# hardcamls/video-coding

Measured on AMD Instinct MI355X. Metric: Mpixel/s decoded (1080p 4:2:0 batch), higher is better.
Workload: dtype int32

## Files before the change

### video-coding_amd/csrc/hvc_capi_reader.hip

```cpp
#include "hvc_batch.h"

static bool same_geometry(const hvc_jpeg_info &a, const hvc_jpeg_info &b) {
    if (a.n_comp != b.n_comp || a.coef_count != b.coef_count || a.width != b.width || a.height != b.height ||
        std::memcmp(a.layout, b.layout, sizeof a.layout))
        return false;
    for (int i = 0; i < a.n_comp; i++) {
        const hvc_jpeg_component &x = a.comp[i], &y = b.comp[i];
        if (x.identifier != y.identifier || x.hscale != y.hscale || x.vscale != y.vscale || x.decoded_width != y.decoded_width ||
            x.decoded_height != y.decoded_height || x.actual_width != y.actual_width || x.actual_height != y.actual_height)
            return false;
    }
    return true;
}

static bool gd_geometry(const hvc_jpeg_info &info0, hvc::HdParams &P) {
    std::memset(&P, 0, sizeof P);
    if (info0.n_comp < 1 || info0.n_comp > 3) return false;
    P.n_comp = info0.n_comp;
    const hvc_jpeg_component &c0 = info0.comp[0];
    if (c0.hscale < 1 || c0.vscale < 1) return false;
    P.mbs_wide = c0.decoded_width / (8 * c0.hscale);
    P.mbs_high = c0.decoded_height / (8 * c0.vscale);
    int base = 0;
    for (int i = 0; i < info0.n_comp; i++) {
        P.comp[i].h = info0.comp[i].hscale;
        P.comp[i].v = info0.comp[i].vscale;
        P.comp[i].bw = info0.layout[i].blocks_w;
        P.comp[i].mcu_base = base;
        P.comp[i].coef_off = info0.layout[i].coef_offset;
        if (P.comp[i].h < 1 || P.comp[i].v < 1) return false;
        if (P.mbs_wide * P.comp[i].h > info0.layout[i].blocks_w || P.mbs_high * P.comp[i].v > info0.layout[i].blocks_h)
            return false;
        if (base + P.comp[i].h * P.comp[i].v > HVC_HD_MAX_MCU_BLOCKS) return false;
        for (int k = 0; k < P.comp[i].h * P.comp[i].v; k++) P.b2comp[base + k] = (unsigned char)i;
        base += P.comp[i].h * P.comp[i].v;
    }
    P.blocks_per_mcu = base;
    const unsigned long long bpf = (unsigned long long)P.mbs_wide * P.mbs_high * base;
    if (bpf == 0 || bpf >= (1ull << 31) || info0.coef_count >= (1ull << 32)) return false;
    P.blocks_per_frame = (unsigned)bpf;
    return true;
}

static void gd_carve_state(hvc::HdParams &P, void *mem, size_t n) {
    unsigned long long *sp = (unsigned long long *)mem;
    P.start_used = sp;
    P.exit_a = sp + n;
    P.exit_b = sp + 2 * n;
    P.exit_c = sp + 3 * n;
    unsigned *up = (unsigned *)(sp + 4 * n);
    P.nblk = up;
    P.list0 = up + n;
    P.list1 = up + 2 * n;
    P.list_n = up + 3 * n;
}

static int gd_upload_tables(hvc_ctx *c, const hvc::HdTables &t, hvc::HdParams &P, hipStream_t st) {
    int r;
    if ((r = grow(c, c->gd_tables, sizeof(hvc::HdTables) + sizeof(hvc::HdSpec) + sizeof(hvc::HdSpecOvf)))) return r;
    hvc::HdSpec spec;
    hvc::HdSpecOvf spec_ovf;
    unsigned char slot[4];
    static const bool classic = std::getenv("HVC_HD_CLASSIC") != nullptr;
    const bool have_spec = hvc::make_spec(t, P.n_comp, spec, slot, P.slot_rep, &spec_ovf) && !classic;
    if (!c->gd_tables_host) c->gd_tables_host.reset(new (std::nothrow) hvc::HdTables);
    if (!c->gd_tables_host) return HVC_E_OUT_OF_MEMORY;
    if (!(c->gd_tables_valid && c->gd_tables_ncomp == P.n_comp && !std::memcmp(c->gd_tables_host.get(), &t, sizeof t))) {
        c->gd_tables_valid = false;
        HIPCHK(c, hipMemcpyAsync(c->gd_tables.p, &t, sizeof t, hipMemcpyHostToDevice, st));
        if (have_spec) {
            HIPCHK(c, hipMemcpyAsync(c->gd_tables.as<char>() + sizeof t, &spec, sizeof spec, hipMemcpyHostToDevice, st));
            HIPCHK(c, hipMemcpyAsync(c->gd_tables.as<char>() + sizeof t + sizeof spec, &spec_ovf, sizeof spec_ovf, hipMemcpyHostToDevice, st));
        }
        HIPCHK(c, hipStreamSynchronize(st));
        std::memcpy(c->gd_tables_host.get(), &t, sizeof t);
        c->gd_tables_ncomp = P.n_comp;
        c->gd_tables_valid = true;
    }
    P.tables = c->gd_tables.as<const hvc::HdTables>();
    P.spec = have_spec ? (const hvc::HdSpec *)(c->gd_tables.as<char>() + sizeof t) : nullptr;
    P.spec_ovf = have_spec ? (const hvc::HdSpecOvf *)(c->gd_tables.as<char>() + sizeof t + sizeof(hvc::HdSpec)) : nullptr;
    P.ftabs = nullptr;
    P.tabset_of = nullptr;
    P.slotmask = P.selmask = 0;
    for (int b = 0; b < P.blocks_per_mcu; b++) {
        P.slotmask |= (unsigned)slot[P.b2comp[b]] << b;
        P.selmask |= (unsigned)slot[P.b2comp[b]] << (2 * b);
    }
    return HVC_OK;
}

static bool gd_lists_per_frame(size_t total_sub, int n_frames) {
    return n_frames >= 1 && n_frames <= 65535 && total_sub / (size_t)n_frames >= 1024;
}

static unsigned gd_component_selmask(const hvc::HdParams &P) {
    unsigned m = 0;
    for (int b = 0; b < P.blocks_per_mcu; b++) m |= (unsigned)P.b2comp[b] << (2 * b);
    return m;
}

static hipError_t gd_enqueue(const hvc::HdParams &P, int rounds, hipStream_t st) {
    hipError_t e = hvc::launch_hd_frame_of(P, st);
    for (int r = 0; r < rounds && e == hipSuccess; r++) e = hvc::launch_hd_round(P, r, st);
    if (e == hipSuccess) e = hvc::launch_hd_finish(P, rounds, st);
    return e;
}
static bool gd_unsettled(unsigned changed_word, int rounds) { return rounds > 1 && changed_word == (unsigned)(rounds - 1); }

static bool call_timing() {
    static const bool on = std::getenv("HVC_CALL_TIMING") != nullptr;
    return on;
}
struct StageClock {
    std::chrono::steady_clock::time_point t0 = std::chrono::steady_clock::now(), last = t0;
    char line[512];
    int n = 0;
    void mark(const char *what) {
        if (!call_timing()) return;
        const auto now = std::chrono::steady_clock::now();
        n += std::snprintf(line + n, sizeof line - (size_t)n, " %s %.1f", what, std::chrono::duration<double, std::micro>(now - last).count());
        if (n > (int)sizeof line - 64) n = (int)sizeof line - 64;
        last = now;
    }
    void done() {
        if (!call_timing()) return;
        std::fprintf(stderr, "hvc call timing (us):%s | total %.1f\n", line, std::chrono::duration<double, std::micro>(last - t0).count());
    }
};

int gpu_entropy_decode(hvc_ctx *c, const uint8_t *const *jpegs, const size_t *sizes, int n_frames, const hvc_jpeg_info &info0,
                       int16_t *d_coefs, size_t coef_fs, int *used_gpu, AfterReader *after) {
    *used_gpu = 0;
    if (after) after->speculated = false;
    StageClock clk;
    std::vector<hvc::HdTables> sets;
    hvc::HdParams P;
// ... 133 lines not shown
        }
        for (size_t k = 0; k < sets.size(); k++) hvc::make_frame_tabs(sets[k], P.n_comp, ftabs[k]);
        const size_t tb = sets.size() * sizeof(hvc::HdFrameTabs);
        if ((r = grow(c, c->gd_ftabs, tb + nU * sizeof(unsigned)))) return r;
        HIPCHK(c, hipMemcpyAsync(c->gd_ftabs.p, ftabs.data(), tb, hipMemcpyHostToDevice, st));
        HIPCHK(c, hipMemcpyAsync(c->gd_ftabs.as<char>() + tb, tabset_of.data(), nU * sizeof(unsigned), hipMemcpyHostToDevice, st));
        P.tables = nullptr;
        P.spec = nullptr;
        P.ftabs = c->gd_ftabs.as<const hvc::HdFrameTabs>();
        P.tabset_of = (const unsigned *)(c->gd_ftabs.as<char>() + tb);
        P.selmask = gd_component_selmask(P);
        if (gd_lists_per_frame(P.total_sub, n_frames)) {
            if ((r = grow(c, c->gd_fcnt, (size_t)HVC_HD_LIST_N * nU * sizeof(unsigned)))) return r;
            P.list_fn = c->gd_fcnt.as<unsigned>();
            for (size_t f = 0; f < (size_t)n_frames; f++) P.max_frame_sub = std::max(P.max_frame_sub, sub_off[(f + 1) * ipf] - sub_off[f * ipf]);
        }
    }
    P.ecs = c->gd_ecs.as<const uint8_t>();
    P.ecs_off = d_ecs_off;
    P.sub_off = d_sub_off;
    P.frame_of = d_frame_of;
    P.coefs = d_coefs;
    P.coef_fs = coef_fs;
    gd_carve_state(P, c->gd_state.p, subs);
    P.frame_blocks = d_frame_blocks;
    P.changed = d_flags;
    P.status = d_flags + 1;
    if (after && after->dc_plane) {
        P.dc_plane = after->dc_plane;
        P.dc_fs = after->dc_fs;
    }
    clk.mark("uploads-enqueued");
    const int first_rounds = 4;
    HIPCHK(c, gd_enqueue(P, first_rounds, st));
    clk.mark("reader-enqueued");
    bool consumer_enqueued = false;
    if (after && after->enqueue) {
        if ((r = after->enqueue())) return r;
        consumer_enqueued = true;
    }
    clk.mark("consumer-enqueued");
    unsigned flags[2] = {0, 0};
    HIPCHK(c, hipMemcpyAsync(flags, P.changed, sizeof flags, hipMemcpyDeviceToHost, st));
    HIPCHK(c, hipStreamSynchronize(st));
    clk.mark("synchronised");
    clk.done();
#ifdef HVC_HD_STATS
    {
        unsigned ln[HVC_HD_LIST_N];
        HIPCHK(c, hipMemcpy(ln, P.list_n, sizeof ln, hipMemcpyDeviceToHost));
        std::fprintf(stderr, "hd stats: %u subsequences; lists", P.total_sub);
        for (int q = 2; q < HVC_HD_LIST_N - 2; q++) std::fprintf(stderr, " %u", ln[q]);
        std::fprintf(stderr, "; k_hd_round walks %u, inner rounds %u; changed %u status %u\n", ln[HVC_HD_LIST_N - 2], ln[HVC_HD_LIST_N - 1], flags[0], flags[1]);
        unsigned long long hs[4];
        hvc::hd_stats_read(hs);
        std::fprintf(stderr, "hd stats: round 0 walked %llu symbols (%.1f a subsequence); 64 x the longest walk of every wavefront: %llu (lanes busy %.1f %%)\n",
                     hs[0], (double)hs[0] / P.total_sub, hs[1], 100.0 * (double)hs[0] / (double)(hs[1] ? hs[1] : 1));
        const unsigned long long own = hs[2] & 0xffffffffull, over = hs[2] >> 32;
        std::fprintf(stderr, "hd stats: write pass %llu symbols inside the lanes' own subsequences + %llu beyond them (%.1f %%); 64 x trips of every wavefront: %llu (lanes busy %.1f %%)\n",
                     own, over, 100.0 * (double)over / (double)(own ? own : 1), hs[3], 100.0 * (double)(own + over) / (double)(hs[3] ? hs[3] : 1));
    }
#endif
    if (gd_unsettled(flags[0], first_rounds)) {
        consumer_enqueued = false;
        const int max_rounds = 48;
        int round = 0;
        HIPCHK(c, hvc::launch_hd_frame_of(P, st));
        for (;; round++) {
            HIPCHK(c, hvc::launch_hd_round(P, round, st));
            if (round >= 4) {
                unsigned changed = 0;
                HIPCHK(c, hipMemcpyAsync(&changed, P.changed, sizeof changed, hipMemcpyDeviceToHost, st));
                HIPCHK(c, hipStreamSynchronize(st));
                if (!gd_unsettled(changed, round + 1)) break;
                if (round >= max_rounds) return HVC_OK;
            }
        }
        HIPCHK(c, hvc::launch_hd_finish(P, round + 1, st));
        HIPCHK(c, hipMemcpyAsync(flags + 1, P.status, sizeof(unsigned), hipMemcpyDeviceToHost, st));
        HIPCHK(c, hipStreamSynchronize(st));
    }
    const unsigned status = flags[1];
    static const bool hd_debug = std::getenv("HVC_HD_DEBUG") != nullptr;
    if (hd_debug) std::fprintf(stderr, "hd debug: frames %d subs %u changed %u status %u\n", P.n_frames, P.total_sub, flags[0], status);
    if (status) return HVC_OK;
    *used_gpu = 1;
    if (after) after->speculated = consumer_enqueued;
    return HVC_OK;
}

int hvc_jpeg_entropy_decode_gpu(hvc_ctx *c, const uint8_t *const *jpegs, const size_t *sizes, int n_frames, int16_t *coefs,
                                size_t coef_fs, int where, hvc_jpeg_info *info, int *used_gpu) try {
    if (!c || !jpegs || !sizes || !coefs || !info || n_frames < 1) return HVC_E_INVALID_ARG;
    if (where != HVC_MEM_HOST && where != HVC_MEM_DEVICE) return HVC_E_INVALID_ARG;
    hvc::RestartScope honour(c->honour_restart);
    int r = hvc_jpeg_read_header(jpegs[0], sizes[0], info);
    if (r) return r;
    if ((n_frames > 1 && coef_fs < info->coef_count) || (coef_fs & 7)) return HVC_E_INVALID_ARG;
    DeviceGuard g(c->device);
    if (!g.ok) return fail_hip(c, hipErrorInvalidDevice);
    int16_t *d = coefs;
    const size_t total = ((size_t)(n_frames - 1) * coef_fs + info->coef_count) * sizeof(int16_t);
    if (where == HVC_MEM_HOST) {
        if ((r = grow(c, c->gd_coefs, total))) return r;
        d = c->gd_coefs.as<int16_t>();
    } else if ((uintptr_t)coefs & 15) {
        return HVC_E_ALIGNMENT;
    }
    int gpu = 0;
    r = gpu_entropy_decode(c, jpegs, sizes, n_frames, *info, d, coef_fs, &gpu);
    if (r) return r;
    if (used_gpu) *used_gpu = gpu;
    if (gpu) {
        if (where == HVC_MEM_HOST) {
            for (int f = 0; f < n_frames; f++)
                HIPCHK(c, hipMemcpyAsync(coefs + (size_t)f * coef_fs, d + (size_t)f * coef_fs, info->coef_count * sizeof(int16_t),
                                         hipMemcpyDeviceToHost, c->stream));
            HIPCHK(c, hipStreamSynchronize(c->stream));
        }
        return HVC_OK;
    }
    std::vector<int16_t> tmp;
    for (int f = 0; f < n_frames; f++) {
        hvc_jpeg_info fi;
        if ((r = hvc_jpeg_read_header(jpegs[f], sizes[f], &fi))) return r;
        if (fi.coef_count != info->coef_count || std::memcmp(fi.layout, info->layout, sizeof fi.layout)) return HVC_E_INVALID_ARG;
        if (where == HVC_MEM_HOST) {
            if ((r = hvc_jpeg_entropy_decode(jpegs[f], sizes[f], &fi, coefs + (size_t)f * coef_fs))) return r;
        } else {
            tmp.resize(info->coef_count);
            if ((r = hvc_jpeg_entropy_decode(jpegs[f], sizes[f], &fi, tmp.data()))) return r;
            HIPCHK(c, hipMemcpyAsync(coefs + (size_t)f * coef_fs, tmp.data(), info->coef_count * sizeof(int16_t),
                                     hipMemcpyHostToDevice, c->stream));
            HIPCHK(c, hipStreamSynchronize(c->stream));
        }
    }
    return HVC_OK;
} HVC_ABI_CATCH

int decode_batch_gpu(hvc_ctx *c, const uint8_t *const *jpegs, const size_t *sizes, int n_frames, int threads, int frames_per_chunk,
                     uint8_t *pixels, size_t pixel_fs, int where, hvc_batch_stats *stats, OutputForm form) {
    if (!c || !jpegs || !sizes || !pixels || n_frames < 0) return HVC_E_INVALID_ARG;
    if (!form.known()) return HVC_E_INVALID_ARG;
    if (where != HVC_MEM_HOST && where != HVC_MEM_DEVICE) return HVC_E_INVALID_ARG;
    if (stats) std::memset(stats, 0, sizeof *stats);
    if (n_frames == 0) return HVC_OK;
    hvc::RestartScope honour(c->honour_restart);
    auto host_pipeline = [&]() {
        return decode_batch_impl(c, jpegs, sizes, n_frames, threads, frames_per_chunk, pixels, pixel_fs, where, stats, form);
    };
    hvc_jpeg_info info0;
    int r = hvc_jpeg_read_header(jpegs[0], sizes[0], &info0);
    if (r) return r;
    form.of(info0);
    if ((r = form.batch_check(pixel_fs))) return r;
    const size_t out_bytes = form.out_bytes;
    hvc::HdParams G;
    hvc::HdTables tables0;
    const unsigned SB = HVC_HD_SUBSEQ_BITS / 8;
    unsigned rst = 0, ipf = 1;
    {
        const bool geo = gd_geometry(info0, G);
        if (geo && hvc::tl_honour_restart) {
            rst = hvc::restart_interval_of(jpegs[0], sizes[0]);
            const unsigned long long mcus = (unsigned long long)G.mbs_wide * (unsigned long long)G.mbs_high;
            if (rst && mcus > rst) {
                const unsigned long long q = (mcus + rst - 1) / rst;
// ... 366 lines not shown
```

### video-coding_amd/csrc/hvc_hdec.h

```cpp
#ifndef HVC_HDEC_H
#define HVC_HDEC_H

#include <hip/hip_runtime.h>
#include <stddef.h>
#include <stdint.h>

#include <vector>

struct hvc_jpeg_info;

namespace hvc {

#define HVC_HD_SUBTABLES 8
#define HVC_HD_OVF 0x3ffu

struct HdTable {
    uint16_t fast[1024];
    uint16_t sub[HVC_HD_SUBTABLES * 64];
};
struct HdOvfRaw {
    uint16_t mincode[6], count[6], valptr[6];
    uint8_t vals[256];
    uint8_t lens[256];
    uint16_t used, pad;
};
struct HdTables {
    HdTable dc[3], ac[3];
    HdOvfRaw ovf_dc[3], ovf_ac[3];
};
struct HdOvf {
    uint16_t mincode[6], count[6], valptr[6], pad[2];
    uint16_t spec[256];
    uint16_t val[256];
};

struct HdSpec {
    uint16_t t[2][2][1024 + HVC_HD_SUBTABLES * 64];
};
struct HdSpecOvf {
    HdOvf o[2][2];
};
bool make_spec(const HdTables &t, int n_comp, HdSpec &out, unsigned char slot_of_comp[4], unsigned char slot_rep[2],
               HdSpecOvf *ovf = nullptr);
bool tables_use_overflow(const HdTables &t, int n_comp);

#define HVC_HD_SPEC_T (1024 + HVC_HD_SUBTABLES * 64)
struct HdFrameTabs {
    uint16_t spec[3][2][HVC_HD_SPEC_T];
    uint16_t val[3][2][HVC_HD_SPEC_T];
    unsigned flags, pad[3];
    HdOvf ovf[3][2];
};
void make_frame_tabs(const HdTables &t, int n_comp, HdFrameTabs &out);

#ifndef HVC_HD_SUBSEQ_BITS
#define HVC_HD_SUBSEQ_BITS 1024
#endif
#define HVC_HD_MAX_MCU_BLOCKS 16
#define HVC_HD_ECS_SLACK 1024
#define HVC_HD_LIST_N 32
#define HVC_HD_STATE_BYTES(n) ((size_t)(n) * (4 * sizeof(unsigned long long) + 3 * sizeof(unsigned)) + HVC_HD_LIST_N * sizeof(unsigned) + 64)

struct HdComp {
    int h, v, bw;
    int mcu_base;
    size_t coef_off;
};

struct HdParams {
    const uint8_t *ecs;
    const unsigned *ecs_off;
    const unsigned *sub_off;
    const unsigned *frame_of;
    const HdTables *tables;
    const HdSpec *spec;
    const HdSpecOvf *spec_ovf;
    const HdFrameTabs *ftabs;
    const unsigned *tabset_of;
    unsigned selmask;
    unsigned slotmask;
    unsigned char slot_rep[2];
    int n_frames;
    unsigned total_sub;
    int n_comp, blocks_per_mcu, mbs_wide, mbs_high;
    unsigned blocks_per_frame;
    unsigned rst_mcus, rst_ipf;
    HdComp comp[4];
    unsigned char b2comp[HVC_HD_MAX_MCU_BLOCKS];
    int16_t *coefs;
    size_t coef_fs;
    unsigned long long *start_used, *exit_a, *exit_b;
    unsigned long long *exit_c;
    unsigned *list0, *list1, *list_n;
    unsigned *list_fn;
    unsigned max_frame_sub;
    int16_t *dcd;
    int16_t *dc_plane;
    size_t dc_fs;
    unsigned *nblk;
    unsigned *frame_blocks;
    unsigned *changed;
    unsigned *status;
};

hipError_t launch_hd_round(const HdParams &P, int round, hipStream_t s);
#ifdef HVC_HD_STATS
void hd_stats_read(unsigned long long out[4]);
#endif
hipError_t launch_hd_frame_of(const HdParams &P, hipStream_t s);
hipError_t launch_hd_finish(const HdParams &P, int rounds_done, hipStream_t s);
bool hd_write2_fits(const HdParams &P);
inline unsigned hd_files(const HdParams &P) { return P.rst_ipf > 1 ? ((unsigned)P.n_frames + P.rst_ipf - 1) / P.rst_ipf : (unsigned)P.n_frames; }

int prepare_gpu_decode(const uint8_t *jpeg, size_t n, const ::hvc_jpeg_info *info, HdTables &t, std::vector<uint8_t> &ecs,
                       bool &gpu_ok);
struct RstUnits {
    unsigned interval, ipf;
    unsigned *off, *len;
};
inline size_t hd_unit_subs(size_t len) { return len ? (len + HVC_HD_SUBSEQ_BITS / 8 - 1) / (HVC_HD_SUBSEQ_BITS / 8) : 1; }
inline size_t hd_unit_slot(size_t len) { return hd_unit_subs(len) * (HVC_HD_SUBSEQ_BITS / 8) + 16; }
int prepare_gpu_decode_to(const uint8_t *jpeg, size_t n, const ::hvc_jpeg_info *info, HdTables &t, uint8_t *dst, size_t cap,
                          size_t *ecs_size, bool &gpu_ok, RstUnits *units = nullptr);
unsigned restart_interval_of(const uint8_t *jpeg, size_t n);


struct WideDc {
    uint32_t block;
    long long dc;
};
extern thread_local bool tl_honour_restart;
struct RestartScope {
    bool prev;
    explicit RestartScope(bool on) : prev(tl_honour_restart) { tl_honour_restart = on; }
    ~RestartScope() { tl_honour_restart = prev; }
};
int entropy_decode_wide(const uint8_t *data, size_t n, const ::hvc_jpeg_info *info, int16_t *coefs, std::vector<WideDc> &wide);
void entropy_decode_wide2(const uint8_t *const data[2], const size_t n[2], const ::hvc_jpeg_info *const info[2], int16_t *const coefs[2],
                          std::vector<WideDc> *const wide[2], int st[2]);

}
#endif
```

### video-coding_amd/csrc/hvc_hdec.hip

```cpp
#include "hvc_hdec_dev.h"

#include <cstdlib>
#include <cstring>
#include <type_traits>

namespace hvc {

using namespace hd_dev;

namespace {

__device__ __forceinline__ bool hd_unsettled(const HdParams &P, int rounds_done) {
    return rounds_done > 1 && *P.changed == (unsigned)(rounds_done - 1);
}

struct FrameRef {
    unsigned file, mcu0, need;
};
__device__ __forceinline__ FrameRef frame_ref(const HdParams &P, unsigned f) {
    FrameRef r{f, 0u, P.blocks_per_frame};
    if (P.rst_ipf > 1u) {
        r.file = f / P.rst_ipf;
        r.mcu0 = (f - r.file * P.rst_ipf) * P.rst_mcus;
        const unsigned left = (unsigned)P.mbs_wide * (unsigned)P.mbs_high - r.mcu0;
        r.need = (left < P.rst_mcus ? left : P.rst_mcus) * (unsigned)P.blocks_per_mcu;
    }
    return r;
}

__device__ __forceinline__ bool one_file(const HdParams &P, unsigned f0, unsigned f1) {
    return f0 == f1 || (P.rst_ipf > 1u && f0 / P.rst_ipf == f1 / P.rst_ipf);
}

__device__ __forceinline__ unsigned be32(const unsigned *g, unsigned i) { return __builtin_bswap32(g[i]); }

__device__ __forceinline__ unsigned lookup(const HdTable &t, unsigned long long w) {
    unsigned e = t.fast[(unsigned)(w >> 54)];
    if (e & 0x8000u) e = t.sub[(e & 0x7fffu) * 64u + ((unsigned)(w >> 48) & 63u)];
    return e;
}

__device__ __forceinline__ int extend(int cat, unsigned code) {
    return (code & (1u << (cat - 1))) ? (int)code : (int)code - (int)((1u << cat) - 1);
}

struct HdGeo {
    int h[4], v[4], bw[4], mcu_base[4];
    unsigned coef_off[4];
    unsigned char b2comp[HVC_HD_MAX_MCU_BLOCKS], b2sx[HVC_HD_MAX_MCU_BLOCKS], b2sy[HVC_HD_MAX_MCU_BLOCKS];
};
__device__ __forceinline__ void load_geo(const HdParams &P, HdGeo &G) {
    if (threadIdx.x < 4) {
        const int i = threadIdx.x;
        G.h[i] = P.comp[i].h;
        G.v[i] = P.comp[i].v;
        G.bw[i] = P.comp[i].bw;
        G.mcu_base[i] = P.comp[i].mcu_base;
        G.coef_off[i] = (unsigned)P.comp[i].coef_off;
    }
    if (threadIdx.x < HVC_HD_MAX_MCU_BLOCKS) {
        const int bb = threadIdx.x, comp = P.b2comp[bb];
        const int r = bb - P.comp[comp].mcu_base, hh = P.comp[comp].h > 0 ? P.comp[comp].h : 1;
        G.b2comp[bb] = (unsigned char)comp;
        G.b2sy[bb] = (unsigned char)(r >= 0 ? r / hh : 0);
        G.b2sx[bb] = (unsigned char)(r >= 0 ? r % hh : 0);
    }
}

template <bool WRITE>
__device__ __forceinline__ void walk(const HdParams &P, const HdGeo &G, const HdTables &T, const unsigned *slot, unsigned base, unsigned limit,
                                     unsigned &p, int &k, int &b, unsigned &nb, unsigned first_block, int16_t *rec,
                                     unsigned &err, int16_t *lb = nullptr, unsigned mcu0 = 0u, unsigned need = 0u) {
    const int B = P.blocks_per_mcu;
    unsigned bi = first_block;
    int16_t *blk = nullptr;
    int lo = k;
    unsigned mx = 0, my = 0;
    if (WRITE) {
        const unsigned mcu = first_block / (unsigned)B + mcu0;
        my = mcu / (unsigned)P.mbs_wide;
        mx = mcu - my * (unsigned)P.mbs_wide;
    }
    auto block_ptr = [&](int bb) -> int16_t * {
        const int comp = G.b2comp[bb];
        return rec + G.coef_off[comp] +
               ((size_t)(my * (unsigned)G.v[comp] + G.b2sy[bb]) * (unsigned)G.bw[comp] + (size_t)(mx * (unsigned)G.h[comp] + G.b2sx[bb])) * 64;
    };
    bool live = WRITE && bi < need;
    if (live) blk = block_ptr(b);
    unsigned off = p - base;
    unsigned wi = (off >> 5) + 2;
    unsigned long long buf = (((unsigned long long)be32(slot, off >> 5) << 32) | be32(slot, (off >> 5) + 1)) << (off & 31u);
    int avail = 64 - (int)(off & 31u);
    unsigned n0 = be32(slot, wi), n1 = be32(slot, min(wi + 1, (unsigned)(S / 32 + 3)));
    int comp = G.b2comp[b];
    const HdTable *dct = &T.dc[comp], *act = &T.ac[comp];
// ... 30 lines not shown
        buf <<= used;
        avail -= used;
        p += (unsigned)used;
        bool end_block = false;
        if (is_dc) {
            if (live) {
                lb[0] = (int16_t)mag;
                if (mag < -32768 || mag > 32767) err |= 2u;
            }
            k = 1;
        } else if (mag == 0 && run == 0) {
            end_block = true;
        } else {
            k += run;
            if (k >= 64) {
                if (live) err |= 1u;
                end_block = true;
            } else {
                if (live && mag) lb[k] = (int16_t)mag;
                k++;
                end_block = k == 64;
            }
        }
        if (end_block) {
            if (live) {
                if (lo == 0) {
                    const uint4 z = make_uint4(0, 0, 0, 0);
#pragma unroll
                    for (int q = 0; q < 8; q++) {
                        reinterpret_cast<uint4 *>(blk)[q] = reinterpret_cast<const uint4 *>(lb)[q];
                        reinterpret_cast<uint4 *>(lb)[q] = z;
                    }
                } else {
                    for (int q = lo; q < 64; q++) {
                        blk[q] = lb[q];
                        lb[q] = 0;
                    }
                }
            }
            lo = 0;
            k = 0;
            b = b + 1 == B ? 0 : b + 1;
            nb++;
            bi++;
            comp = G.b2comp[b];
            dct = &T.dc[comp];
            act = &T.ac[comp];
            if (WRITE && b == 0) {
                mx++;
                if (mx == (unsigned)P.mbs_wide) {
                    mx = 0;
                    my++;
                }
            }
            live = WRITE && bi < need;
            if (live) blk = block_ptr(b);
        }
    }
    if (live)
        for (int q = lo; q < k; q++) blk[q] = lb[q];
}

}


#ifdef HVC_HD_STATS
__device__ unsigned long long g_hd_stats[4];
void hd_stats_read(unsigned long long out[4]) {
    unsigned long long z[4] = {0, 0, 0, 0};
    (void)hipMemcpyFromSymbol(out, HIP_SYMBOL(g_hd_stats), sizeof z);
    (void)hipMemcpyToSymbol(HIP_SYMBOL(g_hd_stats), z, sizeof z);
}
#endif

constexpr int INNER = 24;
template <int MODE>
__global__ __launch_bounds__(256) void k_hd_round(HdParams P, int round) {
    constexpr bool PF = MODE == 2;
    __shared__ __attribute__((aligned(16))) unsigned char Traw[MODE == 0 ? sizeof(HdTables) : sizeof(HdSpec)];
    __shared__ unsigned rows[MODE != 0 ? 256 * SROW + 2 : 1];
    HdTables &T = *reinterpret_cast<HdTables *>(Traw);
    __shared__ HdGeo G;
    __shared__ unsigned long long exits[256];
    load_geo(P, G);
    const int tid = threadIdx.x;
    const unsigned i = blockIdx.x * 256u + (unsigned)tid;
    const bool valid = i < P.total_sub;
    const unsigned f = valid ? P.frame_of[i] : 0u, j = valid ? i - P.sub_off[f] : 0u;
    const unsigned *slot = reinterpret_cast<const unsigned *>(P.ecs + P.ecs_off[f] + (size_t)j * (S / 8));
    const unsigned long long *prev = (round & 1) ? P.exit_a : P.exit_b;
    unsigned long long *cur = (round & 1) ? P.exit_b : P.exit_a;
    const unsigned base = j * (unsigned)S;
    unsigned long long st = pack_state(base, 0, 0), used = 0, ex = 0;
    bool have = false;
    unsigned nb = 0;
    if (valid && round > 0) {
        used = P.start_used[i];
        ex = prev[i];
        nb = P.nblk[i];
        have = true;
        if (j > 0) st = prev[i - 1];
    }
    bool pf_lds = false;
    if (__syncthreads_or(valid && (!have || st != used))) {
        const unsigned *src = MODE == 1 ? reinterpret_cast<const unsigned *>(P.spec) : reinterpret_cast<const unsigned *>(P.tables);
        if (PF) {
            const unsigned i0 = blockIdx.x * 256u, i1 = min(i0 + 256u, P.total_sub) - 1u;
            const unsigned f0 = P.frame_of[i0];
            if (one_file(P, f0, P.frame_of[i1])) {
                const HdFrameTabs &ft = P.ftabs[P.tabset_of[f0]];
                pf_lds = (ft.flags & 1u) != 0u;
                src = reinterpret_cast<const unsigned *>(&ft.spec[0][0][0]);
            }
        }
        if (!PF || pf_lds) {
            unsigned *dst = reinterpret_cast<unsigned *>(Traw);
            for (unsigned q = threadIdx.x; q < sizeof(Traw) / 4; q += 256) dst[q] = src[q];
        }
        __syncthreads();
    }
    bool changed = false;
    for (int inner = 0; inner < INNER; inner++) {
        if (valid && (!have || st != used)) {
            unsigned p = (unsigned)st, err = 0;
            int k = (int)((st >> 32) & 0xffu), b = (int)((st >> 40) & 0xffu);
            nb = 0;
            if (MODE != 0) {
                unsigned *row = rows + tid * SROW;
                stage_row(row, reinterpret_cast<const uint8_t *>(slot));
                auto rd = [row](unsigned q) { return row[q]; };
                const uint16_t *lt = reinterpret_cast<const uint16_t *>(Traw);
                if (MODE == 1) spec_walk<true, true>(rd, row, lt, &P.spec_ovf->o[0][0], P.slotmask, P.blocks_per_mcu, base, p, k, b, nb);
                else if (pf_lds) spec_walk<true, false>(rd, row, lt, &P.ftabs[P.tabset_of[f]].ovf[0][0], selmask_c2_as_c1(P.selmask), P.blocks_per_mcu, base, p, k, b, nb);
                else spec_walk<true, false>(rd, row, &P.ftabs[P.tabset_of[f]].spec[0][0][0], &P.ftabs[P.tabset_of[f]].ovf[0][0], P.selmask, P.blocks_per_mcu, base, p, k, b, nb);
            } else {
                walk<false>(P, G, T, slot, base, base + (unsigned)S, p, k, b, nb, 0, nullptr, err);
            }
            ex = pack_state(p, k, b);
            used = st;
            have = true;
            changed = true;
#ifdef HVC_HD_STATS
            if (round > 0) {
                atomicAdd(&P.list_n[HVC_HD_LIST_N - 2], 1u);
                atomicMax(&P.list_n[HVC_HD_LIST_N - 1], (unsigned)inner + 1u);
            }
#endif
        }
        exits[tid] = ex;
        __syncthreads();
        bool again = false;
        if (valid && j > 0 && tid > 0) {
            st = exits[tid - 1];
            again = st != used;
        }
        if (!__syncthreads_or(again)) break;
    }
    if (valid) {
        cur[i] = ex;
        P.start_used[i] = used;
        P.nblk[i] = nb;
        if (changed && round > 0) *P.changed = (unsigned)round;
    }
}

constexpr int SYNC_ROUNDS = 12, SYNC_ROUNDS_PF = 22;
// ... 97 lines not shown
    const unsigned f = g * ipf, f_end = min(f + ipf, (unsigned)P.n_frames), s0 = P.sub_off[f];
    const unsigned count = round < 2 ? P.sub_off[f_end] - s0 : P.list_fn[(unsigned)round * n_groups + g];
    if (blockIdx.x * (unsigned)SYNC_WG >= count) return;
    const HdFrameTabs &ft = P.ftabs[P.tabset_of[f]];
    const bool pf_lds = (ft.flags & 1u) != 0u;
    if (pf_lds) {
        const unsigned *src = reinterpret_cast<const unsigned *>(&ft.spec[0][0][0]);
        unsigned *dst = reinterpret_cast<unsigned *>(sp);
        for (unsigned i = threadIdx.x; i < sizeof(sp) / 4; i += SYNC_WG) dst[i] = src[i];
        __syncthreads();
    }
    const int wave = threadIdx.x >> 6, lane = threadIdx.x & 63;
    unsigned *row = rows[wave] + lane * SROW;
    const unsigned *list = ((round & 1) ? P.list1 : P.list0) + s0;
    unsigned *next = ((round & 1) ? P.list0 : P.list1) + s0;
    unsigned *next_n = P.list_fn + (unsigned)(round + 1) * n_groups + g;
    const unsigned long long *pe = (round & 1) ? P.exit_b : P.exit_c;
    unsigned long long *ce = (round & 1) ? P.exit_c : P.exit_b;
    int trip = 0;
    for (unsigned tb = blockIdx.x * (unsigned)SYNC_WG; tb < count; tb += gridDim.x * (unsigned)SYNC_WG, trip ^= 1) {
        const unsigned t = tb + (unsigned)threadIdx.x;
        const bool valid = t < count;
        const unsigned i = !valid ? s0 : round < 2 ? s0 + t : list[t];
        const bool push = sync_one<true>(P, round, valid, i, row, sp, pe, ce, pf_lds);
        const unsigned long long m = __ballot(push);
        if (round == 0) continue;
        if (lane == 0) wcount[trip][wave] = (unsigned)__popcll(m);
        __syncthreads();
        if (threadIdx.x == 0) {
            unsigned total = 0;
            for (int q = 0; q < SYNC_WG / 64; q++) total += wcount[trip][q];
            wbase[trip] = total ? atomicAdd(next_n, total) : 0u;
        }
        __syncthreads();
        unsigned at = wbase[trip];
        for (int q = 0; q < wave; q++) at += wcount[trip][q];
        if (push) next[at + (unsigned)__popcll(m & ((1ull << lane) - 1ull))] = i + 1;
    }
}

template <bool PF>
__global__ __launch_bounds__(SYNC_WG) void k_hd_sync_tail(HdParams P, int first_round, int last_round) {
    __shared__ uint16_t sp[PF ? 2 : 2 * 2 * SPEC_T];
    __shared__ unsigned rows[SYNC_WG / 64][64 * SROW + 2];
    __shared__ unsigned cnt_s[2];
    if (!PF) {
        const unsigned *src = reinterpret_cast<const unsigned *>(P.spec);
        unsigned *dst = reinterpret_cast<unsigned *>(sp);
        for (unsigned i = threadIdx.x; i < sizeof(HdSpec) / 4; i += SYNC_WG) dst[i] = src[i];
    }
    if (threadIdx.x == 0) {
        cnt_s[first_round & 1] = P.list_n[first_round];
        cnt_s[(first_round + 1) & 1] = 0;
    }
    __syncthreads();
    const int wave = threadIdx.x >> 6, lane = threadIdx.x & 63;
    unsigned *row = rows[wave] + lane * SROW;
    for (int round = first_round; round <= last_round; round++) {
        const unsigned count = cnt_s[round & 1];
        if (count == 0) break;
        const unsigned *list = (round & 1) ? P.list1 : P.list0;
        unsigned *next = (round & 1) ? P.list0 : P.list1;
        const unsigned long long *pe = (round & 1) ? P.exit_b : P.exit_c;
        unsigned long long *ce = (round & 1) ? P.exit_c : P.exit_b;
        for (unsigned t0 = (unsigned)wave * 64u; t0 < count; t0 += (unsigned)SYNC_WG) {
            const unsigned t = t0 + (unsigned)lane;
            const bool valid = t < count;
            const unsigned i = valid ? list[t] : 0u;
            const bool push = sync_one<PF>(P, round, valid, i, row, sp, pe, ce);
            const unsigned long long m = __ballot(push);
            if (m) {
                unsigned at = 0;
                if (lane == 0) at = atomicAdd(&cnt_s[(round + 1) & 1], (unsigned)__popcll(m));
                at = __shfl(at, 0);
                if (push) next[at + (unsigned)__popcll(m & ((1ull << lane) - 1ull))] = i + 1;
            }
        }
        __syncthreads();
        if (threadIdx.x == 0) cnt_s[round & 1] = 0;
        __syncthreads();
    }
}

__global__ __launch_bounds__(1024) void k_hd_scan(HdParams P) {
    __shared__ unsigned wsum[16];
    __shared__ unsigned carry_s;
    const int frame = blockIdx.x, lane = threadIdx.x, wave = lane >> 6, wl = lane & 63;
    unsigned *d = P.nblk + P.sub_off[frame];
    const unsigned n = P.sub_off[frame + 1] - P.sub_off[frame];
    if (lane == 0) carry_s = 0;
    __syncthreads();
    for (unsigned base = 0; base < n; base += 1024) {
        const unsigned idx = base + (unsigned)lane;
        const unsigned v = idx < n ? d[idx] : 0u;
        unsigned incl = v;
#pragma unroll
        for (int o = 1; o < 64; o <<= 1) {
            const unsigned t = __shfl_up(incl, o);
            if (wl >= o) incl += t;
        }
        if (wl == 63) wsum[wave] = incl;
        __syncthreads();
        unsigned wbase = 0;
        for (int q = 0; q < wave; q++) wbase += wsum[q];
        const unsigned excl = carry_s + wbase + incl - v;
        if (idx < n) d[idx] = excl;
        __syncthreads();
        if (lane == 1023) carry_s = excl + v;
        __syncthreads();
    }
    if (lane == 0) {
        P.frame_blocks[frame] = carry_s;
        if (carry_s < frame_ref(P, (unsigned)frame).need) atomicOr(P.status, 4u);
    }
}

__global__ __launch_bounds__(256) void k_hd_write(HdParams P, int final_round) {
    __shared__ HdTables T;
    __shared__ HdGeo G;
    __shared__ uint4 lbuf[256 * 8];
    load_geo(P, G);
    {
        const unsigned *src = reinterpret_cast<const unsigned *>(P.tables);
        unsigned *dst = reinterpret_cast<unsigned *>(&T);
        for (unsigned i = threadIdx.x; i < sizeof(HdTables) / 4; i += 256) dst[i] = src[i];
#pragma unroll
        for (int q = 0; q < 8; q++) lbuf[threadIdx.x * 8 + q] = make_uint4(0, 0, 0, 0);
    }
    const unsigned i = blockIdx.x * 256u + threadIdx.x;
    const bool valid = i < P.total_sub;
    const unsigned f = valid ? P.frame_of[i] : 0u, j = valid ? i - P.sub_off[f] : 0u;
    const unsigned *slot = reinterpret_cast<const unsigned *>(P.ecs + P.ecs_off[f] + (size_t)j * (S / 8));
    __syncthreads();
    if (hd_unsettled(P, final_round)) return;
    if (!valid) return;
    const unsigned first_block = P.nblk[i];
    const FrameRef R = frame_ref(P, f);
    if (first_block >= R.need) return;
    const unsigned long long st = P.start_used[i];
    unsigned p = (unsigned)st;
    int k = (int)((st >> 32) & 0xffu), b = (int)((st >> 40) & 0xffu);
    unsigned nb = 0, err = 0;
    if ((unsigned)b != first_block % (unsigned)P.blocks_per_mcu) {
        atomicOr(P.status, 8u);
        return;
    }
    const unsigned base = j * (unsigned)S;
    walk<true>(P, G, T, slot, base, base + (unsigned)S, p, k, b, nb, first_block, P.coefs + (size_t)R.file * P.coef_fs, err,
               reinterpret_cast<int16_t *>(lbuf + threadIdx.x * 8), R.mcu0, R.need);
    const unsigned long long *fin = (final_round & 1) ? P.exit_a : P.exit_b;
    if (pack_state(p, k, b) != fin[i]) err |= 8u;
    if (err) atomicOr(P.status, err);
}

constexpr int WR_EXTRA = 3;
#ifndef HVC_WR_BATCH
#define HVC_WR_BATCH 12
#endif
constexpr int WR_BATCH = HVC_WR_BATCH;

template <bool PF, bool GBITS, int WG>
__global__ __launch_bounds__(WG) void k_hd_write2(HdParams P, int final_round) {
    __shared__ uint16_t tv[2 * 2 * SPEC_T];
    __shared__ HdGeo G;
    __shared__ unsigned rows[GBITS ? 1 : (WG + WR_EXTRA + 2) * SROW];
    __shared__ uint4 lbuf[WG * 8];
    __shared__ uint2 flist[WG / 64][64];
    load_geo(P, G);
    {
        for (int sl = 0; sl < (PF ? 0 : 2); sl++)
            for (int cls = 0; cls < 2; cls++) {
                const HdTable *src_t = cls ? &P.tables->ac[P.slot_rep[sl]] : &P.tables->dc[P.slot_rep[sl]];
                const uint16_t *src = reinterpret_cast<const uint16_t *>(src_t);
                for (unsigned i = threadIdx.x; i < sizeof(HdTable) / 2; i += WG) tv[(sl * 2 + cls) * SPEC_T + i] = (uint16_t)val_entry(src[i], cls == 0, i >= 1024u);
            }
#pragma unroll
        for (int q = 0; q < 8; q++) lbuf[threadIdx.x * 8 + q] = make_uint4(0, 0, 0, 0);
    }
    const int tid = threadIdx.x, wave = tid >> 6, lane = tid & 63;
    const unsigned i = blockIdx.x * (unsigned)WG + (unsigned)tid;
    const bool valid = i < P.total_sub;
    const unsigned f = valid ? P.frame_of[i] : 0u, j = valid ? i - P.sub_off[f] : 0u;
    if (hd_unsettled(P, final_round)) return;
    bool pf_lds = false;
    if (PF) {
        const unsigned i0 = blockIdx.x * (unsigned)WG, i1 = min(i0 + (unsigned)WG, P.total_sub) - 1u;
        const unsigned f0 = P.frame_of[i0];
        if (one_file(P, f0, P.frame_of[i1])) {
            const HdFrameTabs &ft = P.ftabs[P.tabset_of[f0]];
            if (ft.flags & 1u) {
                pf_lds = true;
                const unsigned *src = reinterpret_cast<const unsigned *>(&ft.val[0][0][0]);
                unsigned *dst = reinterpret_cast<unsigned *>(tv);
                for (unsigned q = threadIdx.x; q < sizeof(tv) / 4; q += WG) dst[q] = src[q];
            }
        }
    }
    if (!GBITS) {
        if (valid) stage_row(rows + tid * SROW, P.ecs + P.ecs_off[f] + (size_t)j * (S / 8));
        if (tid < WR_EXTRA) {
            const unsigned i2 = blockIdx.x * (unsigned)WG + (unsigned)WG + (unsigned)tid;
            if (i2 < P.total_sub) {
                const unsigned f2 = P.frame_of[i2];
                stage_row(rows + (WG + tid) * SROW, P.ecs + P.ecs_off[f2] + (size_t)(i2 - P.sub_off[f2]) * (S / 8));
            }
        }
    }
    __syncthreads();
    const unsigned *row = rows + (GBITS ? 0 : tid * SROW);
    const unsigned *gbits = reinterpret_cast<const unsigned *>(P.ecs + P.ecs_off[f] + (size_t)j * (S / 8));
    auto rd = [&](unsigned q) -> unsigned { return GBITS ? __builtin_bswap32(gbits[q]) : row[q + (q ? (q - 1u) >> 5 : 0u)]; };
    auto rd1 = [&](unsigned q) -> unsigned { return GBITS ? __builtin_bswap32(gbits[q]) : row[q + ((q - 1u) >> 5)]; };
    static_assert(S == 1024, "rd(): S / 32 dwords per row");
    int16_t *const nowhere = reinterpret_cast<int16_t *>(&flist[wave][lane]);
    int16_t *const lb = reinterpret_cast<int16_t *>(lbuf + tid * 8);
    const int B = P.blocks_per_mcu;
    const unsigned base = j * (unsigned)S, limit = base + (unsigned)S, hard = limit + (unsigned)(WR_EXTRA * S);
    unsigned bi = valid ? P.nblk[i] : 0xffffffffu;
    const FrameRef R = frame_ref(P, f);
    bool act = valid && bi < R.need;
    const unsigned long long st = act ? P.start_used[i] : 0ull;
    const unsigned p0 = act ? (unsigned)st : base;
    int k = (int)((st >> 32) & 0xffu), b = (int)((st >> 40) & 0xffu);
    unsigned err = 0;
    if (act && (unsigned)b != bi % (unsigned)B) {
        err |= 8u;
        act = false;
    }
    bool live = act && k == 0;
    const unsigned mcu = (act ? bi : 0u) / (unsigned)B + R.mcu0;
    unsigned my = mcu / (unsigned)P.mbs_wide, mx = mcu - my * (unsigned)P.mbs_wide;
    const unsigned frame_unit0 = (unsigned)(((size_t)R.file * P.coef_fs) >> 3);
    auto block_no = [&](int bb) -> unsigned {
        const int comp = G.b2comp[bb];
        return frame_unit0 + (G.coef_off[comp] >> 3) +
               ((my * (unsigned)G.v[comp] + G.b2sy[bb]) * (unsigned)G.bw[comp] + (mx * (unsigned)G.h[comp] + G.b2sx[bb])) * 8u;
    };
    unsigned mm = ~(p0 - base + 31u);
    const unsigned l0 = (p0 - base + 31u) >> 5;
    unsigned hi = l0 ? rd(l0 - 1u) : 0u, lo = rd(l0), nx = rd(l0 + 1u);
    auto pos = [&]() -> unsigned { return base + ~mm - 31u; };
    auto mm_of = [&](unsigned p) -> unsigned { return ~(p - base + 31u); };
    auto decode_and_store = [&](const uint16_t *const tvb, const HdOvf *const ovf, const unsigned selmask) {
    const uint16_t *bt = tvb + ((selmask >> (2 * b)) & 3u) * (2 * SPEC_T);
    const uint16_t *bt_ac = bt + SPEC_T;
    const unsigned long long fin_i = valid ? ((final_round & 1) ? P.exit_a : P.exit_b)[i] : 0ull;
    const unsigned mm_limit = mm_of(limit), mm_hard = mm_of(hard);
    unsigned watch = mm_limit;
    unsigned cur_block = live ? block_no(b) : 0u;
#ifdef HVC_HD_STATS
    unsigned st_sym = 0, st_trips = 0;
#endif
    while (__any(act)) {
        unsigned npend = 0;
        if (act) for (;;) {
            const unsigned w = __builtin_amdgcn_alignbit(hi, lo, mm);
            const uint16_t *t = k ? bt_ac : bt;
            const HdSymbol sy = val_symbol(w, t, ovf, selmask, b, k);
            const unsigned used = sy.used;
            const int kn = sy.kn;
            const bool wrong = sy.wrong, end_block = sy.end_block;
            *((live && !wrong) ? lb + kn - 1 : nowhere) = (int16_t)sy.mag;
            k = end_block ? 64 : kn;
            const unsigned mn = mm - used;
            const bool refill = ((mn ^ mm) >> 5) != 0u;
            mm = mn;
            if (!GBITS) {
                hi = refill ? lo : hi;
                lo = refill ? nx : lo;
                nx = rd1((31u - mn) >> 5);
            } else if (refill) {
                hi = lo;
                lo = nx;
                nx = rd1((31u - mn) >> 5);
            }
            if ((live && wrong) || mm <= watch) {
                if (live && wrong) atomicOr(P.status, 1u);
                if (mm <= watch) {
                    if (watch == mm_limit) {
                        if (pack_state(pos(), end_block ? 0 : k, end_block ? (b + 1 == B ? 0 : b + 1) : b) != fin_i) atomicOr(P.status, 8u);
                        watch = mm_hard;
                        if (!end_block && !live) k = 65;
                    } else {
                        atomicOr(P.status, 1u);
                        k = 65;
                    }
                }
            }
            npend += (unsigned)__popcll(__ballot(k == 64));
#ifdef HVC_HD_STATS
            st_sym += mm > mm_limit ? 1u : 0x10000u;
            st_trips += (unsigned)__popcll(__ballot(true)) ? 1u : 0u;
#endif
            if (k >= 64 || npend >= (unsigned)WR_BATCH) break;
        }
        if (k == 65) act = false;
        const bool pending = act && k == 64;
        if (__any(pending)) {
            const bool flush = pending && live;
            const unsigned long long m = __ballot(flush);
            asm volatile("" ::: "memory");
            const unsigned n = (unsigned)__popcll(m);
            if (flush) {
                flist[wave][__popcll(m & ((1ull << lane) - 1ull))] = make_uint2(cur_block, (unsigned)(wave * 64 + lane));
                P.dcd[(size_t)f * P.blocks_per_frame + bi] = lb[0];
            }
            for (unsigned g = 0; g < n; g += 8) {
                const unsigned en = g + ((unsigned)lane >> 3);
                if (en < n) {
                    const uint2 fe = flist[wave][en];
                    uint4 *src = lbuf + fe.y * 8u + ((unsigned)lane & 7u);
                    reinterpret_cast<uint4 *>(P.coefs)[(size_t)fe.x + ((unsigned)lane & 7u)] = *src;
                    *src = make_uint4(0, 0, 0, 0);
                }
            }
            asm volatile("" ::: "memory");
            if (pending) {
                k = 0;
                b = b + 1 == B ? 0 : b + 1;
                bi++;
                live = bi < R.need;
                bt = tvb + ((selmask >> (2 * b)) & 3u) * (2 * SPEC_T);
                bt_ac = bt + SPEC_T;
                if (b == 0) {
                    mx++;
                    if (mx == (unsigned)P.mbs_wide) {
                        mx = 0;
                        my++;
                    }
// ... 99 lines not shown
        if (val) val[q] = (uint16_t)val_entry(e, dc, q >= 1024);
    }
}

static void convert_ovf(const HdOvfRaw &src, bool dc, HdOvf &o) {
    std::memset(&o, 0, sizeof o);
    for (int i = 0; i < 6; i++) {
        o.mincode[i] = src.mincode[i];
        o.count[i] = src.used ? src.count[i] : (uint16_t)0;
        o.valptr[i] = src.valptr[i];
    }
    for (int k = 0; k < 256; k++) {
        const unsigned len = src.lens[k], v = src.vals[k];
        uint16_t sp = 1, vl = 1;
        if (len) {
            const HdTable *none = nullptr;
            (void)none;
            const unsigned e = (len << 8) | v;
            if (dc) sp = (uint16_t)(v > 16 ? len : (len + v) | (1u << 6));
            else {
                const unsigned size = v & 15u, run = v >> 4;
                sp = (!size && !run) ? (uint16_t)(len | (64u << 6)) : (uint16_t)((len + size) | ((run + 1u) << 6));
            }
            vl = (uint16_t)val_entry(e, dc, true);
        }
        o.spec[k] = sp;
        o.val[k] = vl;
    }
}

bool tables_use_overflow(const HdTables &t, int n_comp) {
    for (int c = 0; c < n_comp && c < 3; c++)
        if (t.ovf_dc[c].used || t.ovf_ac[c].used) return true;
    return false;
}

bool make_spec(const HdTables &t, int n_comp, HdSpec &out, unsigned char slot_of_comp[4], unsigned char slot_rep[2], HdSpecOvf *ovf) {
    if (n_comp < 1 || n_comp > 3) return false;
    int rep[2] = {0, -1};
    for (int c = 0; c < 4; c++) slot_of_comp[c] = 0;
    for (int c = 1; c < n_comp; c++) {
        auto same = [&](int a) { return !std::memcmp(&t.dc[c], &t.dc[a], sizeof(HdTable)) && !std::memcmp(&t.ac[c], &t.ac[a], sizeof(HdTable)); };
        if (same(rep[0])) continue;
        if (rep[1] < 0) rep[1] = c;
        if (!same(rep[1])) return false;
        slot_of_comp[c] = 1;
    }
    slot_rep[0] = 0;
    slot_rep[1] = (unsigned char)(rep[1] < 0 ? 0 : rep[1]);
    std::memset(&out, 0, sizeof out);
    if (ovf) std::memset(ovf, 0, sizeof *ovf);
    for (int sl = 0; sl < 2; sl++) {
        if (rep[sl] < 0) continue;
        convert_table(t.dc[rep[sl]], true, out.t[sl][0], nullptr);
        convert_table(t.ac[rep[sl]], false, out.t[sl][1], nullptr);
        if (ovf) {
            convert_ovf(t.ovf_dc[rep[sl]], true, ovf->o[sl][0]);
            convert_ovf(t.ovf_ac[rep[sl]], false, ovf->o[sl][1]);
        }
    }
    return true;
}

void make_frame_tabs(const HdTables &t, int n_comp, HdFrameTabs &out) {
    out.flags = (n_comp < 3 || (!std::memcmp(&t.dc[2], &t.dc[1], sizeof(HdTable)) && !std::memcmp(&t.ac[2], &t.ac[1], sizeof(HdTable)))) ? 1u : 0u;
    out.pad[0] = out.pad[1] = out.pad[2] = 0;
    for (int c = 0; c < 3; c++) {
        const int s = c < n_comp ? c : 0;
        convert_table(t.dc[s], true, out.spec[c][0], out.val[c][0]);
        convert_table(t.ac[s], false, out.spec[c][1], out.val[c][1]);
        convert_ovf(t.ovf_dc[s], true, out.ovf[c][0]);
        convert_ovf(t.ovf_ac[s], false, out.ovf[c][1]);
    }
}

__global__ __launch_bounds__(256) void k_hd_frame_of(HdParams P) {
    const unsigned f = blockIdx.x, end = P.sub_off[f + 1];
    unsigned *frame_of = const_cast<unsigned *>(P.frame_of);
    for (unsigned q = P.sub_off[f] + threadIdx.x; q < end; q += 256u) frame_of[q] = f;
    if (f == 0) {
        if (threadIdx.x < HVC_HD_LIST_N) P.list_n[threadIdx.x] = 0u;
        if (threadIdx.x == 0) {
            *P.changed = 0u;
            *P.status = 0u;
        }
    }
    if (P.list_fn && threadIdx.x < HVC_HD_LIST_N) P.list_fn[threadIdx.x * (unsigned)P.n_frames + f] = 0u;
}

hipError_t launch_hd_frame_of(const HdParams &P, hipStream_t s) {
    if (P.total_sub == 0 || P.n_frames <= 0) return hipSuccess;
    hipLaunchKernelGGL(k_hd_frame_of, dim3((unsigned)P.n_frames), dim3(256), 0, s, P);
    return hipGetLastError();
}

template <bool PF>
static hipError_t launch_hd_round_t(const HdParams &P, int round, hipStream_t s) {
    if (round == 0 && (PF || P.spec)) {
        const unsigned all = (P.total_sub + (unsigned)SYNC_WG - 1u) / (unsigned)SYNC_WG;
        if (P.total_sub <= SYNC_TAIL_MAX_SUB) {
            for (int r = 0; r < SYNC_TAIL_FROM; r++) hipLaunchKernelGGL(k_hd_sync<PF>, dim3(all), dim3(SYNC_WG), 0, s, P, r);
            hipLaunchKernelGGL(k_hd_sync_tail<PF>, dim3(1), dim3(SYNC_WG), 0, s, P, SYNC_TAIL_FROM, SYNC_TAIL_FROM + 200);
            return hipGetLastError();
        }
        static const int rounds = [] {
            const char *v = getenv(PF ? "HVC_HD_SYNC_ROUNDS_PF" : "HVC_HD_SYNC_ROUNDS");
            const int most = PF ? SYNC_ROUNDS_PF : SYNC_ROUNDS, n = v ? atoi(v) : most;
            return n < 2 ? 2 : n > HVC_HD_LIST_N - 4 ? HVC_HD_LIST_N - 4 : n;
        }();
        if (PF && P.list_fn && P.max_frame_sub) {
            const unsigned per_frame = (P.max_frame_sub + (unsigned)SYNC_WG - 1u) / (unsigned)SYNC_WG;
            for (int r = 0; r < rounds; r++) hipLaunchKernelGGL(k_hd_sync_pf, dim3(per_frame, hd_files(P)), dim3(SYNC_WG), 0, s, P, r);
            return hipGetLastError();
        }
        for (int r = 0; r < rounds; r++) {
            const unsigned grid = r < 2 ? all : min(all, r < 4 ? 2048u : 512u);
            hipLaunchKernelGGL(k_hd_sync<PF>, dim3(grid), dim3(SYNC_WG), 0, s, P, r);
        }
        return hipGetLastError();
    }
    if (PF) hipLaunchKernelGGL(k_hd_round<2>, dim3((P.total_sub + 255u) / 256u), dim3(256), 0, s, P, round);
    else if (P.spec) hipLaunchKernelGGL(k_hd_round<1>, dim3((P.total_sub + 255u) / 256u), dim3(256), 0, s, P, round);
    else hipLaunchKernelGGL(k_hd_round<0>, dim3((P.total_sub + 255u) / 256u), dim3(256), 0, s, P, round);
    return hipGetLastError();
}

hipError_t launch_hd_round(const HdParams &P, int round, hipStream_t s) {
    if (P.total_sub == 0) return hipSuccess;
    return P.ftabs ? launch_hd_round_t<true>(P, round, s) : launch_hd_round_t<false>(P, round, s);
}

bool hd_write2_fits(const HdParams &P) { return (unsigned long long)hd_files(P) * P.coef_fs < (1ull << 35); }

hipError_t launch_hd_finish(const HdParams &P, int rounds_done, hipStream_t s) {
    if (P.total_sub == 0) return hipSuccess;
    hipLaunchKernelGGL(k_hd_scan, dim3((unsigned)P.n_frames), dim3(1024), 0, s, P);
    HdParams Q = P;
    static const int wr_mode = [] { const char *v = getenv("HVC_WR_MODE"); return v ? atoi(v) : 0; }();
    auto write2 = [&](auto pf) {
        constexpr bool PFv = decltype(pf)::value;
        if (wr_mode == 1) hipLaunchKernelGGL((k_hd_write2<PFv, true, 512>), dim3((P.total_sub + 511u) / 512u), dim3(512), 0, s, P, rounds_done);
        else if (wr_mode == 2) hipLaunchKernelGGL((k_hd_write2<PFv, true, 256>), dim3((P.total_sub + 255u) / 256u), dim3(256), 0, s, P, rounds_done);
        else hipLaunchKernelGGL((k_hd_write2<PFv, false, 256>), dim3((P.total_sub + 255u) / 256u), dim3(256), 0, s, P, rounds_done);
    };
    if (P.ftabs) {
        if (!P.dcd || !hd_write2_fits(P)) return hipErrorInvalidValue;
        write2(std::true_type{});
    } else if (P.spec && P.dcd && hd_write2_fits(P)) {
        write2(std::false_type{});
    } else {
        Q.dcd = nullptr;
        hipLaunchKernelGGL(k_hd_write, dim3((P.total_sub + 255u) / 256u), dim3(256), 0, s, P, rounds_done);
    }
    hipLaunchKernelGGL(k_hd_dc, dim3((unsigned)P.n_comp, (unsigned)P.n_frames), dim3(1024), 0, s, Q, rounds_done);
    return hipGetLastError();
}

}
```

Measured before the change: 1.340 million.

## Add device-side convergence check to skip redundant Huffman sync rounds

After the round-0 synchronization kernels, a new check kernel verifies that every subsequence's start state matches its predecessor's exit state and records a resync flag if any mismatch remains. Later round kernels early-exit when the flag is clear, and the finish/write kernels choose the exit array based on that flag. This aims to remove the cost of the further self-synchronization rounds (kernel launches and host round-trips still occur, but the kernels return immediately). It adds one extra check kernel pass over the state arrays per batch.

```diff
diff --git a/video-coding_amd/csrc/hvc_capi_reader.hip b/video-coding_amd/csrc/hvc_capi_reader.hip
--- a/video-coding_amd/csrc/hvc_capi_reader.hip
+++ b/video-coding_amd/csrc/hvc_capi_reader.hip
@@ -53,6 +53,7 @@
     P.list0 = up + n;
     P.list1 = up + 2 * n;
     P.list_n = up + 3 * n;
+    P.resync = P.list_n + HVC_HD_LIST_N;
 }
 
 static int gd_upload_tables(hvc_ctx *c, const hvc::HdTables &t, hvc::HdParams &P, hipStream_t st) {
@@ -352,7 +353,11 @@
     }
     const unsigned status = flags[1];
     static const bool hd_debug = std::getenv("HVC_HD_DEBUG") != nullptr;
-    if (hd_debug) std::fprintf(stderr, "hd debug: frames %d subs %u changed %u status %u\n", P.n_frames, P.total_sub, flags[0], status);
+    if (hd_debug) {
+        unsigned resync = 0;
+        HIPCHK(c, hipMemcpy(&resync, P.resync, sizeof resync, hipMemcpyDeviceToHost));
+        std::fprintf(stderr, "hd debug: frames %d subs %u changed %u status %u resync %u\n", P.n_frames, P.total_sub, flags[0], status, resync);
+    }
     if (status) return HVC_OK;
     *used_gpu = 1;
     if (after) after->speculated = consumer_enqueued;
diff --git a/video-coding_amd/csrc/hvc_hdec.h b/video-coding_amd/csrc/hvc_hdec.h
--- a/video-coding_amd/csrc/hvc_hdec.h
+++ b/video-coding_amd/csrc/hvc_hdec.h
@@ -59,7 +59,7 @@
 #define HVC_HD_MAX_MCU_BLOCKS 16
 #define HVC_HD_ECS_SLACK 1024
 #define HVC_HD_LIST_N 32
-#define HVC_HD_STATE_BYTES(n) ((size_t)(n) * (4 * sizeof(unsigned long long) + 3 * sizeof(unsigned)) + HVC_HD_LIST_N * sizeof(unsigned) + 64)
+#define HVC_HD_STATE_BYTES(n) ((size_t)(n) * (4 * sizeof(unsigned long long) + 3 * sizeof(unsigned)) + (HVC_HD_LIST_N + 1) * sizeof(unsigned) + 64)
 
 struct HdComp {
     int h, v, bw;
@@ -100,6 +100,7 @@
     unsigned *nblk;
     unsigned *frame_blocks;
     unsigned *changed;
+    unsigned *resync;
     unsigned *status;
 };
 
diff --git a/video-coding_amd/csrc/hvc_hdec.hip b/video-coding_amd/csrc/hvc_hdec.hip
--- a/video-coding_amd/csrc/hvc_hdec.hip
+++ b/video-coding_amd/csrc/hvc_hdec.hip
@@ -12,6 +12,12 @@
 
 __device__ __forceinline__ bool hd_unsettled(const HdParams &P, int rounds_done) {
     return rounds_done > 1 && *P.changed == (unsigned)(rounds_done - 1);
+}
+
+__device__ __forceinline__ bool hd_rounds_idle(const HdParams &P) { return (P.spec || P.ftabs) && *P.resync == 0u; }
+__device__ __forceinline__ const unsigned long long *hd_final_exits(const HdParams &P, int final_round) {
+    const unsigned long long *const a = P.exit_a, *const b = P.exit_b;
+    return ((final_round & 1) || hd_rounds_idle(P)) ? a : b;
 }
 
 struct FrameRef {
@@ -208,6 +214,7 @@
     HdTables &T = *reinterpret_cast<HdTables *>(Traw);
     __shared__ HdGeo G;
     __shared__ unsigned long long exits[256];
+    if (MODE != 0 && round > 0 && hd_rounds_idle(P)) return;
     load_geo(P, G);
     const int tid = threadIdx.x;
     const unsigned i = blockIdx.x * 256u + (unsigned)tid;
@@ -471,6 +478,39 @@
     }
 }
 
+constexpr int CHECK_WG = 256;
+template <bool V16>
+__global__ __launch_bounds__(CHECK_WG) void k_hd_check(HdParams P, int round) {
+    const unsigned long long *prev = (round & 1) ? P.exit_a : P.exit_b;
+    const unsigned n = P.total_sub;
+    const int lane = threadIdx.x & 63;
+    bool bad = false;
+    for (unsigned tb = blockIdx.x * (2u * CHECK_WG); tb < n; tb += gridDim.x * (2u * CHECK_WG)) {
+        const unsigned i0 = tb + 2u * threadIdx.x;
+        const bool have0 = i0 < n, have1 = i0 + 1u < n;
+        unsigned long long su0 = 0, su1 = 0, ex0 = 0, ex1 = 0;
+        unsigned f0 = 0, f1 = 0;
+        if (V16 && have1) {
+            const ulonglong2 su = *reinterpret_cast<const ulonglong2 *>(P.start_used + i0);
+            const ulonglong2 ex = *reinterpret_cast<const ulonglong2 *>(prev + i0);
+            su0 = su.x, su1 = su.y, ex0 = ex.x, ex1 = ex.y;
+        } else if (have0) {
+            su0 = P.start_used[i0];
+            ex0 = prev[i0];
+            if (have1) su1 = P.start_used[i0 + 1u], ex1 = prev[i0 + 1u];
+        }
+        if (have0) f0 = P.frame_of[i0];
+        if (have1) f1 = P.frame_of[i0 + 1u];
+        unsigned long long exm = __shfl_up(ex1, 1);
+        unsigned fm = __shfl_up(f1, 1);
+        if (lane == 0 && have0 && i0 > 0u) exm = prev[i0 - 1u], fm = P.frame_of[i0 - 1u];
+        const unsigned long long first = pack_state(0u, 0, 0);
+        bad |= have0 && su0 != ((i0 == 0u || fm != f0) ? first : exm);
+        bad |= have1 && su1 != (f0 != f1 ? first : ex0);
+    }
+    if (__any(bad) && lane == 0) *P.resync = (unsigned)round;
+}
+
 __global__ __launch_bounds__(1024) void k_hd_scan(HdParams P) {
     __shared__ unsigned wsum[16];
     __shared__ unsigned carry_s;
@@ -537,8 +577,7 @@
     const unsigned base = j * (unsigned)S;
     walk<true>(P, G, T, slot, base, base + (unsigned)S, p, k, b, nb, first_block, P.coefs + (size_t)R.file * P.coef_fs, err,
                reinterpret_cast<int16_t *>(lbuf + threadIdx.x * 8), R.mcu0, R.need);
-    const unsigned long long *fin = (final_round & 1) ? P.exit_a : P.exit_b;
-    if (pack_state(p, k, b) != fin[i]) err |= 8u;
+    if (pack_state(p, k, b) != hd_final_exits(P, final_round)[i]) err |= 8u;
     if (err) atomicOr(P.status, err);
 }
 
@@ -633,7 +672,7 @@
     auto decode_and_store = [&](const uint16_t *const tvb, const HdOvf *const ovf, const unsigned selmask) {
     const uint16_t *bt = tvb + ((selmask >> (2 * b)) & 3u) * (2 * SPEC_T);
     const uint16_t *bt_ac = bt + SPEC_T;
-    const unsigned long long fin_i = valid ? ((final_round & 1) ? P.exit_a : P.exit_b)[i] : 0ull;
+    const unsigned long long fin_i = valid ? hd_final_exits(P, final_round)[i] : 0ull;
     const unsigned mm_limit = mm_of(limit), mm_hard = mm_of(hard);
     unsigned watch = mm_limit;
     unsigned cur_block = live ? block_no(b) : 0u;
@@ -899,6 +938,7 @@
         if (threadIdx.x < HVC_HD_LIST_N) P.list_n[threadIdx.x] = 0u;
         if (threadIdx.x == 0) {
             *P.changed = 0u;
+            *P.resync = 0u;
             *P.status = 0u;
         }
     }
@@ -908,6 +948,13 @@
 hipError_t launch_hd_frame_of(const HdParams &P, hipStream_t s) {
     if (P.total_sub == 0 || P.n_frames <= 0) return hipSuccess;
     hipLaunchKernelGGL(k_hd_frame_of, dim3((unsigned)P.n_frames), dim3(256), 0, s, P);
+    return hipGetLastError();
+}
+
+static hipError_t launch_hd_check(const HdParams &P, hipStream_t s) {
+    const unsigned per_wg = 2u * (unsigned)CHECK_WG, wgs = (P.total_sub + per_wg - 1u) / per_wg, grid = wgs < 2048u ? wgs : 2048u;
+    if ((((uintptr_t)P.start_used | (uintptr_t)P.exit_a) & 15u) == 0u) hipLaunchKernelGGL(k_hd_check<true>, dim3(grid), dim3(CHECK_WG), 0, s, P, 1);
+    else hipLaunchKernelGGL(k_hd_check<false>, dim3(grid), dim3(CHECK_WG), 0, s, P, 1);
     return hipGetLastError();
 }
 
@@ -944,7 +991,9 @@
 
 hipError_t launch_hd_round(const HdParams &P, int round, hipStream_t s) {
     if (P.total_sub == 0) return hipSuccess;
-    return P.ftabs ? launch_hd_round_t<true>(P, round, s) : launch_hd_round_t<false>(P, round, s);
+    const hipError_t e = P.ftabs ? launch_hd_round_t<true>(P, round, s) : launch_hd_round_t<false>(P, round, s);
+    if (e == hipSuccess && round == 0 && (P.ftabs || P.spec)) return launch_hd_check(P, s);
+    return e;
 }
 
 bool hd_write2_fits(const HdParams &P) { return (unsigned long long)hd_files(P) * P.coef_fs < (1ull << 35); }
```

Result: no change. 1.342 million, median of 3 (+0.2%).
